# GestaltCogTeam/STEP

Measured on AMD Instinct MI355X. Metric: training windows/sec on PEMS04, horizon-12 MAE parity, 1/2/4/8 MI355X, higher is better.
Workload: dtype f16 (TSFormer Q/K/weights) + bf16 (P, V, GraphWaveNet / graph-learner GEMMs) operands, f32 accumulate

## Files before the change

### step_amd/csrc/gemm.hip

```cpp
#include "common.h"
#include "step_internal.h"

namespace {

constexpr int BK = 32;

template <typename T>
__device__ __forceinline__ float ld_elem(const void* p, long idx) {
    if constexpr (sizeof(T) == 2) {
        return bf16_bits_to_f32(((const uint16_t*)p)[idx]);
    } else {
        return ((const float*)p)[idx];
    }
}

template <int BM, int BN, int WM, int WN, typename TA, typename TB>
__global__ __launch_bounds__(256) void gemm_f32mfma_kernel(StepGemm g) {
    constexpr int TM = BM / WM / 32;
    constexpr int TN = BN / WN / 32;
    constexpr int LDA = BM + 4;
    constexpr int LDB = BN + 4;
    __shared__ __attribute__((aligned(16))) float As[BK * LDA];
    __shared__ __attribute__((aligned(16))) float Bs[BK * LDB];

// ... 396 lines not shown
    }
    if (g.splitk < 1) g.splitk = 1;
    if (g.splitk == 1 && direct_eligible(g)) return launch_direct(g, st);
    if (g.splitk > 1) {
        STEP_REQUIRE(g.accumulate == 2, "step_gemm: split-K needs accumulate==2 (atomic) and a pre-zeroed/accumulating C");
    }
    STEP_REQUIRE(!(g.accumulate == 2 && (g.bias || g.relu)), "step_gemm: bias/relu epilogue not available with atomic accumulate");
    if (g.N <= 32 && g.M > 64) return launch<128, 32, 4, 1>(g, st);
    if (g.M <= 32 && g.N > 64) return launch<32, 128, 1, 4>(g, st);
    if (g.M <= 64 || g.N <= 64) return launch<64, 64, 2, 2>(g, st);
    long tiles128 = (long)cdiv(g.M, 128) * cdiv(g.N, 128) * g.batch * g.splitk;
    if (tiles128 < 256) return launch<64, 64, 2, 2>(g, st);
    return launch<128, 128, 2, 2>(g, st);
}

int step_gemm_launch_fused(StepGemm g, const GemmFused& fused, hipStream_t st) {
    STEP_REQUIRE(g.M > 0 && g.N > 0 && g.K >= 0 && g.batch == 1 && g.A && g.B && g.C, "step_gemm(fused): bad descriptor");
    STEP_REQUIRE(fused.channels > 0 && fused.period > 0 && (long)fused.channels * fused.period == g.N, "step_gemm(fused): N != channels * period");
    if (g.scn == 0) g.scn = 1;
    if (g.splitk < 1) g.splitk = 1;
    if (g.c_nscale) STEP_REQUIRE(g.c_nshift && g.c_mvec && g.c_nperiod == fused.period, "step_gemm(fused): column affine must use the same period");
    if (g.compute_bf16) return step_gemm_bf16_launch(g, st, &fused);
    const int rc = step_gemm_f32_fast_launch(g, st, &fused);
    if (rc == -1) { step_set_error("step_gemm(fused): operands do not qualify for the staged path"); return STEP_ERR_ARG; }
    return rc;
}

extern "C" int step_gemm(const StepGemm* g, void* stream) {
    STEP_REQUIRE(g != nullptr, "step_gemm: null descriptor");
    return step_gemm_launch(*g, (hipStream_t)stream);
// ... 2 lines not shown
```

### step_amd/csrc/gemm_bf16.hip

```cpp
#include "common.h"
#include "step_internal.h"

namespace {

constexpr int BK = 32;
constexpr int PITCH = BK * 2 + 16;

typedef __attribute__((ext_vector_type(4))) float f32x4v;
typedef __attribute__((ext_vector_type(4))) __bf16 bf16x4;

typedef __attribute__((ext_vector_type(2))) float f32x2v;
typedef __attribute__((ext_vector_type(2))) __bf16 bf16x2v;
__device__ __forceinline__ uint32_t pack2(float a, float b) {
    uint32_t r;
    asm("v_cvt_pk_bf16_f32 %0, %1, %2" : "=v"(r) : "v"(a), "v"(b));
    return r;
}
__device__ __forceinline__ uint2 pack4(float a, float b, float c, float d) { return make_uint2(pack2(a, b), pack2(c, d)); }
__device__ __forceinline__ uint2 pack4(const float (&v)[4]) { return pack4(v[0], v[1], v[2], v[3]); }
__device__ __forceinline__ uint16_t bf16_of(float x) {
    return __builtin_bit_cast(uint16_t, (__bf16)x);
}
template <typename T>
__device__ __forceinline__ float ld1(const void* p, long idx) {
// ... 189 lines not shown

enum { KC_F32 = 0, KC_BF16 = 1, MC_F32 = 2, MC_BF16 = 3 };
constexpr int FBK = 64;
constexpr int FPITCH = FBK * 2 + 8;
constexpr int FPITCH32 = FBK * 4 + 16;

struct FastArgs {
    const GemmKSeg* ktab;
    int ktab_per;
    int a_klog, b_klog, b_nlog;
    int xcd_swizzle;
    int wide_store;
    int m_fast;
    long split_stride;
    GemmFused fu;
};

static int wide_store_ok(const StepGemm& g, bool force = false) {
    return g.accumulate != 2 && !g.a_rowsum && g.c_nblk == 0 && g.scn == 1 && g.N % 4 == 0 && g.ldc % 4 == 0 && g.scb % 4 == 0 &&
           g.scb1 % 4 == 0 && ((uintptr_t)g.C & 15) == 0 && (force || (long)g.M * g.N * g.batch >= (4L << 20));
}

__device__ __forceinline__ long remap(int i, int lg, long stride) {
    return (long)(i >> lg) * stride + (i & ((1 << lg) - 1));
}

template <int MODE, int BR>
struct Stage {
    static constexpr int NV = MODE == KC_F32 ? BR * FBK / 4 / 256 : (MODE == KC_BF16 ? BR * FBK / 8 / 256 : (MODE == MC_F32 ? BR * FBK / 16 / 256 : (BR * FBK / 32 + 255) / 256));
    static constexpr int NR = (MODE == MC_F32 || MODE == MC_BF16) ? NV * 4 : NV;
// ... 178 lines not shown
                *(uint2*)(d + (2 * p + 1) * FPITCH) = make_uint2((d0 >> 16) | (d1 & 0xffff0000u), (d2 >> 16) | (d3 & 0xffff0000u));
            }
        }
    } else {
#pragma unroll
        for (int r = 0; r < s.NV; ++r) {
            const int e = tid + r * 256;
            char* d = lds + ((e % (BR / 4)) * 4) * FPITCH + (e / (BR / 4)) * 8;
#pragma unroll
            for (int i = 0; i < 4; ++i)
                *(uint2*)(d + i * FPITCH) = pack4(s.f[r * 4][i], s.f[r * 4 + 1][i], s.f[r * 4 + 2][i], s.f[r * 4 + 3][i]);
        }
    }
}

template <int BM, int BN, int AMODE, int BMODE, bool F32C, bool KTAB = false, bool FUSED = false>
__global__ __launch_bounds__(256) void gemm_fast_kernel(StepGemm g, FastArgs fa) {
    static_assert(!KTAB || (AMODE == KC_F32 && BMODE == KC_F32), "segmented contraction: k-contiguous f32 blocks on both sides");
    constexpr int TM = BM / 64, TN = BN / 64;
    constexpr int PITCH_ = F32C ? FPITCH32 : FPITCH;
    constexpr int BUF = (BM + BN) * PITCH_;
    __shared__ __attribute__((aligned(16))) char lds[2 * BUF];

    const int tid = threadIdx.x, lane = tid & 63, wave = tid >> 6;
    const int wr = wave >> 1, wc = wave & 1;
    unsigned bx = blockIdx.x, by = blockIdx.y, bz = blockIdx.z;
    if (fa.xcd_swizzle) {
        const unsigned gx = gridDim.x, lin = bx + gx * (by + gridDim.y * bz);
        const unsigned q = lin >> 3, j = q / gx, grp = (lin & 7u) + 8u * j;
        bx = q - j * gx; by = grp % gridDim.y; bz = grp / gridDim.y;
    } else if (fa.m_fast) {
// ... 281 lines not shown
            }
        }
        if (fu.dotw) {
            float q4[4] = {dw[0], dm[0], dw[1], dm[1]};
#pragma unroll
            for (int i = 0; i < 4; ++i) q4[i] = wave_sum(q4[i]);
            if (lane == 0) { fred[wave][0] = q4[0]; fred[wave][1] = q4[1]; fred[wave][2] = q4[2]; fred[wave][3] = q4[3]; }
            __syncthreads();
            if (tid < 4) {
                const int c = c_lo + (tid >> 1);
                if (c < C) atomicAdd(fu.dots + 2 * c + (tid & 1), fred[0][tid] + fred[1][tid] + fred[2][tid] + fred[3][tid]);
            }
        }
        return;
    }
    if constexpr (BM * (BN + 4) * 4 <= 2 * BUF)
    if (fa.wide_store) {
        constexpr int TP = BN + 4;
        static_assert(BM * TP * 4 <= 2 * BUF, "staging tile must fit in the operand buffers");
        float* tile = (float*)lds;
        __syncthreads();
#pragma unroll
        for (int i = 0; i < TM; ++i)
#pragma unroll
            for (int j = 0; j < TN; ++j) {
                const int cn = wc * (TN * 32) + j * 32 + r, gn = n0 + cn;
                const GemmColAffine ca = gemm_col_affine(g, gn < g.N ? gn : 0);
                const float bv = (g.bias != nullptr && gn < g.N) ? g.bias[gn] : 0.f;
#pragma unroll
                for (int e = 0; e < 16; ++e) {
// ... 66 lines not shown
    if (bmode == KC_F32) gemm_fast_kernel<BM, BN, AMODE, KC_F32, false><<<grid, 256, 0, st>>>(g, fa);
    else if (bmode == KC_BF16) gemm_fast_kernel<BM, BN, AMODE, KC_BF16, false><<<grid, 256, 0, st>>>(g, fa);
    else if (bmode == MC_F32) gemm_fast_kernel<BM, BN, AMODE, MC_F32, false><<<grid, 256, 0, st>>>(g, fa);
    else {
        if constexpr (AMODE != KC_BF16) gemm_fast_kernel<BM, BN, AMODE, MC_BF16, false><<<grid, 256, 0, st>>>(g, fa);
        else { step_set_error("step_gemm: an n-contiguous bf16 B operand needs an f32 A operand"); return STEP_ERR_ARG; }
    }
    STEP_LAUNCH_CHECK("step_gemm(bf16 fast)");
    return STEP_OK;
}
template <int BM, int BN>
int launch_fast(const StepGemm& g, const FastArgs& fa_in, int amode, int bmode, hipStream_t st) {
    dim3 grid(cdiv(g.N + (g.a_rowsum ? 1 : 0), BN), cdiv(g.M, BM), g.batch * g.splitk);
    FastArgs fa = fa_in;
    fa.xcd_swizzle = grid.x >= 2 && (grid.y * grid.z) % 8 == 0 && (long)g.M * g.K * g.batch >= (8L << 20);
    if (amode == KC_F32) return launch_fast_b<BM, BN, KC_F32>(g, fa, bmode, grid, st);
    if (amode == KC_BF16) return launch_fast_b<BM, BN, KC_BF16>(g, fa, bmode, grid, st);
    return launch_fast_b<BM, BN, MC_F32>(g, fa, bmode, grid, st);
}
template <int BM, int BN>
int launch_fast_fused(const StepGemm& g, const FastArgs& fa_in, int amode, int bmode, hipStream_t st) {
    dim3 grid(cdiv(g.N, BN), cdiv(g.M, BM), 1);
    FastArgs fa = fa_in;
    static const bool m_fast_on = []() { const char* e = getenv("STEP_GEMM_M_FAST"); return !e || atoi(e) != 0; }();
    fa.m_fast = m_fast_on && grid.y >= 2 && grid.y <= 64 && (long)g.N * g.K * (g.b_bf16 ? 2 : 4) >= (16L << 20);
    if (amode == KC_F32 && bmode == MC_BF16) gemm_fast_kernel<BM, BN, KC_F32, MC_BF16, false, false, true><<<grid, 256, 0, st>>>(g, fa);
    else if (amode == KC_F32 && bmode == KC_F32) gemm_fast_kernel<BM, BN, KC_F32, KC_F32, false, false, true><<<grid, 256, 0, st>>>(g, fa);
    else if (amode == KC_F32 && bmode == MC_F32) gemm_fast_kernel<BM, BN, KC_F32, MC_F32, false, false, true><<<grid, 256, 0, st>>>(g, fa);
    else if (amode == MC_F32 && bmode == MC_F32) gemm_fast_kernel<BM, BN, MC_F32, MC_F32, false, false, true><<<grid, 256, 0, st>>>(g, fa);
    else { step_set_error("step_gemm(fused): operand layout not instantiated"); return STEP_ERR_ARG; }
// ... 45 lines not shown
    const long i0 = batch0 ? b % batch0 : b, i1 = batch0 ? b / batch0 : 0;
    atomicAdd(C + i0 * scb + i1 * scb1 + m * ldc + n * scn, s);
}
}

static int auto_splitk(int M, int N, int K, int batch, bool fast) {
    const int bk = fast ? FBK : BK;
    long tiles = fast ? (long)cdiv(M, 128) * cdiv(N, 128) * batch : (long)cdiv(M, 64) * cdiv(N, 64) * batch;
    static const int split_target = []() { const char* e = getenv("STEP_GEMM_SPLIT_TARGET"); return e ? atoi(e) : 768; }();
    long want = ((fast ? split_target : 1024) + tiles - 1) / tiles;
    long maxs = cdiv(K, bk) / 4;
    return (int)(want < 1 ? 1 : (want > maxs ? (maxs < 1 ? 1 : maxs) : want));
}
int step_gemm_auto_splitk(int M, int N, int K, int batch) { return auto_splitk(M, N, K, batch, true); }

int step_gemm_bf16_launch(StepGemm g, hipStream_t st, const GemmFused* fused) {
    FastArgs fa;
    memset(&fa, 0, sizeof(fa));
    if (fused) fa.fu = *fused;
    int dummy;
    const int amode = fast_mode(g.A, g.a_bf16, g.sam, g.sak, g.sab, g.sab1, g.a_kblk, g.a_kstride, 0, 0, &fa.a_klog, &dummy);
    const int bmode = fast_mode(g.B, g.b_bf16, g.sbn, g.sbk, g.sbb, g.sbb1, g.b_kblk, g.b_kstride, g.b_nblk, g.b_nstride, &fa.b_klog,
                                &fa.b_nlog);
    const bool fast = amode >= 0 && amode != MC_BF16 && bmode >= 0 && !(g.a_kscale && (amode != KC_F32 || g.a_kperiod < FBK)) &&
                !(g.a_rowsum && (bmode == KC_BF16 || bmode == MC_BF16)) && !(bmode == MC_BF16 && g.N % 8);
    fa.wide_store = wide_store_ok(g, fused != nullptr);
    if (fused) STEP_REQUIRE(fast && fa.wide_store && !g.bias && !g.relu && g.batch == 1 && g.splitk <= 1 &&
                            ((fused->flags & (GEMM_FUSED_FFN_FWD | GEMM_FUSED_MASKNZ | GEMM_FUSED_BF16OUT)) ? (g.accumulate == 0 && !fused->dotw && !fused->bnx && !g.c_nscale) :
                             (fused->flags & GEMM_FUSED_INTERLEAVED) ? (128 % fused->channels == 0 && fused->channels % 8 == 0 && g.N % 8 == 0 && g.ldc % 8 == 0 &&
                                                                       ((((uintptr_t)fused->bnx) | ((uintptr_t)g.C)) & 15) == 0 && !fused->dotw) : fused->period >= 128),
                            "step_gemm: the fused DGL epilogues need the staged path with a wide-store result (aligned dense C, period >= 128)");
    if (g.splitk < 0) {
        STEP_REQUIRE(g.accumulate == 2, "step_gemm: automatic split-K needs accumulate==2");
        g.splitk = auto_splitk(g.M, g.N, g.K, g.batch, fast);
    }
    if (g.splitk < 1) g.splitk = 1;
    if (g.splitk > 1) STEP_REQUIRE(g.accumulate == 2, "step_gemm: split-K needs accumulate==2");
    STEP_REQUIRE(!(g.accumulate == 2 && (g.bias || g.relu)), "step_gemm: bias/relu epilogue not available with atomic accumulate");
    long tiles128 = (long)cdiv(g.M, 128) * cdiv(g.N, 128) * g.batch * g.splitk;
    const bool big = g.M > 64 && g.N > 64 && tiles128 >= 512;
    static const bool use_ws = []() { const char* e = getenv("STEP_GEMM_SPLITK_WS"); return !e || atoi(e) != 0; }();
    const StepGemm orig = g;
    bool ws_reduce = false;
    if (use_ws && fast && !fused && g.splitk > 1 && g.splitk_ws && !g.c_nblk && !g.c_nscale && (((uintptr_t)g.splitk_ws) & 15) == 0 &&
        (long)g.M * g.N * g.batch * g.splitk <= g.splitk_ws_floats) {
        const long mn = (long)g.M * g.N;
// ... 83 lines not shown
```

### step_amd/csrc/gwnet.hip

```cpp
#include "common.h"
#include "step_internal.h"
#include <vector>

namespace {

constexpr int C = 32, CAT = 224, CS = 256, CE = 512, OUT = 12, NL = 8, HID = 96;
constexpr int TIN[NL] = {13, 12, 10, 9, 7, 6, 4, 3};
constexpr int DIL[NL] = {1, 2, 1, 2, 1, 2, 1, 2};
constexpr int TOUT[NL] = {12, 10, 9, 7, 6, 4, 3, 1};

__global__ void start_conv_kernel(const float* __restrict__ hist, int B, int N, int Cin, const float* __restrict__ w,
                                  const float* __restrict__ b, float* __restrict__ x0) {
    long idx = (long)blockIdx.x * 256 + threadIdx.x;
    long total = (long)B * N * 13 * C;
    if (idx >= total) return;
    int c = idx % C, t = (idx / C) % 13;
    long bn = idx / (C * 13);
    int n = bn % N, bb = bn / N;
    float v = b[c];
    if (t >= 1) {
        const float* src = hist + (((long)bb * 12 + (t - 1)) * N + n) * Cin;
        v += w[c * 2] * src[0] + w[c * 2 + 1] * src[1];
    }
    x0[idx] = v;
// ... 86 lines not shown
}
__global__ void stacks_to_bf16_kernel(const float* __restrict__ P, const float* __restrict__ PT, long rows, int N, int N8,
                                      uint16_t* __restrict__ P16, uint16_t* __restrict__ PT16) {
    long idx = (long)blockIdx.x * 256 + threadIdx.x;
    if (idx >= rows * (N8 / 2)) return;
    const long row = idx / (N8 / 2);
    const int j = (int)(idx % (N8 / 2)) * 2;
    const float* src = blockIdx.y ? PT : P;
    uint16_t* dst = blockIdx.y ? PT16 : P16;
    const float a = j < N ? src[row * N + j] : 0.f, b = j + 1 < N ? src[row * N + j + 1] : 0.f;
    typedef __attribute__((ext_vector_type(2))) float f2;
    typedef __attribute__((ext_vector_type(2))) __bf16 b2;
    f2 t = {a, b};
    *(uint32_t*)(dst + row * N8 + j) = __builtin_bit_cast(uint32_t, __builtin_convertvector(t, b2));
}
__global__ __launch_bounds__(256) void slots_to_bf16T_kernel(const float* __restrict__ cat, int slot0, int sstep, int B, int N, int T, int N8,
                                                             uint16_t* __restrict__ XT) {
    __shared__ float tile[64][33];
    const int v0 = blockIdx.x * 64, t = blockIdx.y, src = blockIdx.z / B, b = blockIdx.z % B;
    const int slot = slot0 + sstep * src;
    const int c = threadIdx.x & 31, r = threadIdx.x >> 5;
    for (int i = r; i < 64; i += 8) {
        const int v = v0 + i;
        tile[i][c] = v < N ? cat[(((long)b * N + v) * T + t) * CAT + slot * C + c] : 0.f;
    }
    __syncthreads();
    const int cc = threadIdx.x >> 3, g8 = (threadIdx.x & 7) * 8;
    if (v0 + g8 < N8) {
        float v8[8];
#pragma unroll
        for (int j = 0; j < 8; ++j) v8[j] = tile[g8 + j][cc];
        *(bf16x8*)(XT + (((long)blockIdx.z * T + t) * C + cc) * N8 + v0 + g8) = pack8(v8);
    }
}
__global__ void sum_batches_kernel(const float* __restrict__ x, long n, int B, float* __restrict__ out) {
    long idx = (long)blockIdx.x * 256 + threadIdx.x;
    if (idx >= n) return;
    float s = 0.f;
    for (int b = 0; b < B; ++b) s += x[(long)b * n + idx];
    out[idx] = s;
}
__global__ __launch_bounds__(256) void row_dot_kernel(const float* __restrict__ dP, const float* __restrict__ P, int N,
                                                      float* __restrict__ out) {
    __shared__ float red[4];
    const long row = blockIdx.x;
    float s = 0.f;
    for (int j = threadIdx.x; j < N; j += 256) s += dP[row * N + j] * P[row * N + j];
    s = wave_sum(s);
// ... 170 lines not shown
    __shared__ double tot[64];
    if (threadIdx.x < 64) tot[threadIdx.x] = gather_sum(bn.sums, threadIdx.x);
    __syncthreads();
    if (threadIdx.x < 32) {
        const int c = threadIdx.x;
        co[c] = (float)(tot[c] / bn.count); co[32 + c] = (float)(tot[32 + c] / bn.count); co[64 + c] = bn.gamma[c] * bn.stat[96 + c];
        if (blockIdx.x == 0) { bn.dgamma[c] += (float)tot[32 + c]; bn.dbeta[c] += (float)tot[c]; }
    }
    __syncthreads();
}

template <bool BF16>
__global__ __launch_bounds__(256) void tcn_fwd_kernel(const float* __restrict__ src, BnFwd bn, long npos, int Tin, int Tout, int dil,
                                                      const float* __restrict__ wcat, const float* __restrict__ bcat,
                                                      float* __restrict__ tf, float* __restrict__ sg, float* __restrict__ cat,
                                                      float* __restrict__ zlast, int layer) {
    __shared__ float st[128];
    if (bn.stat) bn_fwd_stats(bn, st);
    const int lane = threadIdx.x & 63, wave = threadIdx.x >> 6, col = lane & 31, h = lane >> 5;
    const long r0 = ((long)blockIdx.x * 4 + wave) * 32;
    if (r0 >= npos) return;
    long p = r0 + col;
    if (p >= npos) p = npos - 1;
    const long bn_ = p / Tout;
    const long xrow = bn_ * Tin + (p - bn_ * Tout);
    float a[4][8], bf[4][8], bg[4][8];
#pragma unroll
    for (int q = 0; q < 4; ++q) {
        load8h(src + (xrow + (q >> 1) * dil) * C + 16 * (q & 1), h, a[q]);
        load8h(wcat + col * 64 + 16 * q, h, bf[q]);
        load8h(wcat + (32 + col) * 64 + 16 * q, h, bg[q]);
    }
    if (bn.stat) {
#pragma unroll
        for (int q = 0; q < 4; ++q)
#pragma unroll
            for (int j = 0; j < 8; ++j) { const int c = chan8h(q & 1, h, j); a[q][j] = a[q][j] * st[c] + st[32 + c]; }
    }
    f32x16 af, ag;
#pragma unroll
    for (int e = 0; e < 16; ++e) { af[e] = 0.f; ag[e] = 0.f; }
#pragma unroll
    for (int q = 0; q < 4; ++q) { mma16<BF16>(af, a[q], bf[q]); mma16<BF16>(ag, a[q], bg[q]); }
    const float b_f = bcat[col], b_g = bcat[32 + col];
#pragma unroll
    for (int e = 0; e < 16; ++e) {
        const long pe = r0 + (e & 3) + 8 * (e >> 2) + 4 * h;
        if (pe >= npos) continue;
        const float f = tanhf(af[e] + b_f);
        const float g = 1.f / (1.f + __expf(-(ag[e] + b_g)));
        tf[pe * C + col] = f; sg[pe * C + col] = g;
        cat[pe * CAT + col] = f * g;
        const long bne = pe / Tout;
        if (pe - bne * Tout == Tout - 1) zlast[bne * CS + layer * C + col] = f * g;
    }
}

template <bool BF16>
__global__ __launch_bounds__(256) void mix_fwd_kernel(const float* __restrict__ cat, const float* __restrict__ w,
                                                      const float* __restrict__ bias, XIn x, long npos, int Tin, int Tout, int dil,
                                                      float drop_p, uint32_t seed_lo, uint32_t seed_hi, uint32_t layer,
                                                      float* __restrict__ mask, float* __restrict__ y, double* __restrict__ sums,
                                                      const StepDynState* __restrict__ dyn) {
    if (dyn) { const uint64_t sx = dyn->seed_xor; seed_lo ^= (uint32_t)sx; seed_hi ^= (uint32_t)(sx >> 32); }
    __shared__ float red[4][64];
    __shared__ float bsum[64];
    const int lane = threadIdx.x & 63, wave = threadIdx.x >> 6, ln = lane & 15, kg = lane >> 4;
    const long r0 = ((long)blockIdx.x * 4 + wave) * 16;
    float s1[2] = {0.f, 0.f}, s2[2] = {0.f, 0.f};
    if (r0 < npos) {
// ... 49 lines not shown
        for (int half = 0; half < 2; ++half) {
            s1[half] += __shfl_xor(s1[half], 16, 64); s2[half] += __shfl_xor(s2[half], 16, 64);
            s1[half] += __shfl_xor(s1[half], 32, 64); s2[half] += __shfl_xor(s2[half], 32, 64);
        }
    }
    if (kg == 0) { red[wave][ln] = s1[0]; red[wave][16 + ln] = s1[1]; red[wave][32 + ln] = s2[0]; red[wave][48 + ln] = s2[1]; }
    __syncthreads();
    if (threadIdx.x < 64) bsum[threadIdx.x] = red[0][threadIdx.x] + red[1][threadIdx.x] + red[2][threadIdx.x] + red[3][threadIdx.x];
    __syncthreads();
    add_block_sums(sums, bsum);
}

template <bool BF16>
__global__ __launch_bounds__(256) void mix_bwd_kernel(const float* __restrict__ dy, const float* __restrict__ y, BnBwd bn,
                                                      const float* __restrict__ mask, const float* __restrict__ wT, long npos,
                                                      float* __restrict__ dres, float* __restrict__ dh, float* __restrict__ dcat) {
    __shared__ float co[96];
    bn_bwd_coef(bn, co);
    const int lane = threadIdx.x & 63, wave = threadIdx.x >> 6, col = lane & 31, h = lane >> 5;
    const long r0 = ((long)blockIdx.x * 4 + wave) * 32;
    if (r0 >= npos) return;
    const long p = r0 + col;
    const bool ok = p < npos;
    float a[2][8];
#pragma unroll
    for (int q = 0; q < 2; ++q) {
        float d8[8] = {0.f, 0.f, 0.f, 0.f, 0.f, 0.f, 0.f, 0.f}, y8[8] = {0.f, 0.f, 0.f, 0.f, 0.f, 0.f, 0.f, 0.f}, m8[8] = {1.f, 1.f, 1.f, 1.f, 1.f, 1.f, 1.f, 1.f};
        if (ok) {
            load8h(dy + p * C + 16 * q, h, d8); load8h(y + p * C + 16 * q, h, y8);
            if (mask) load8h(mask + p * C + 16 * q, h, m8);
        }
#pragma unroll
        for (int j = 0; j < 8; ++j) {
            const int c = chan8h(q, h, j);
            const float xhat = (y8[j] - bn.stat[64 + c]) * bn.stat[96 + c];
            const float d = ok ? co[64 + c] * (d8[j] - co[c] - xhat * co[32 + c]) : 0.f;
            d8[j] = d;
            a[q][j] = d * m8[j];
        }
        if (ok) { store8h(dres + p * C + 16 * q, h, d8); store8h(dh + p * C + 16 * q, h, a[q]); }
    }
#pragma unroll
    for (int slot = 0; slot < 7; ++slot) {
        float b[2][8];
#pragma unroll
        for (int q = 0; q < 2; ++q) load8h(wT + (slot * C + col) * C + 16 * q, h, b[q]);
        f32x16 acc;
#pragma unroll
        for (int e = 0; e < 16; ++e) acc[e] = 0.f;
#pragma unroll
        for (int q = 0; q < 2; ++q) mma16<BF16>(acc, a[q], b[q]);
#pragma unroll
        for (int e = 0; e < 16; ++e) {
            const long pe = r0 + (e & 3) + 8 * (e >> 2) + 4 * h;
            if (pe < npos) dcat[pe * CAT + slot * C + col] = acc[e];
        }
    }
}

constexpr int TB_ROWS = 64;
template <bool BF16>
__global__ __launch_bounds__(256) void tcn_bwd_kernel(const float* __restrict__ dcat, const float* __restrict__ dzlast, int layer,
                                                      const float* __restrict__ tf, const float* __restrict__ sg,
                                                      const float* __restrict__ wcatT, const float* __restrict__ dres, long BN, int Tin,
                                                      int Tout, int dil, float* __restrict__ dpre, float* __restrict__ dx,
                                                      const float* __restrict__ yprev, const float* __restrict__ statprev,
                                                      double* __restrict__ sums) {
    __shared__ float dxs[TB_ROWS][65];
    __shared__ float red[8][64];
    __shared__ float bsum[64];
    const int G = TB_ROWS / Tout, R = G * Tout;
// ... 147 lines not shown
inline dim3 g1(long n) { return dim3((unsigned)((n + 255) / 256)); }

struct Carver {
    float* base;
    long used = 0;
    explicit Carver(float* b) : base(b) {}
    float* take(long n) {
        float* p = base ? base + used : nullptr;
        used += (n + 3) & ~3L;
        return p;
    }
};

static inline int n8(int N) { return (N + 7) & ~7; }
static inline bool hop_transposed_operand(int N) {
    static const int min_n = []() { const char* e = getenv("STEP_HOP_XT_MIN_N"); return e ? atoi(e) : 768; }();
    return N >= min_n;
}

struct Saved {
    float *x0, *cat[NL], *tf[NL], *sg[NL], *y[NL], *mask[NL], *bnstat[NL], *zlast;
    float *Pstk, *PTstk, *Pa, *Madp, *rs, *cs;
    uint16_t *P16, *PT16;
    float *skip, *h1, *h2, *xh, *e1;
    long total;
};
Saved carve_saved(float* base, int B, int N, bool dropout) {
    Carver cv(base);
    Saved s;
    const long BN = (long)B * N;
    s.x0 = cv.take(BN * TIN[0] * C);
// ... 14 lines not shown
    s.Madp = cv.take((long)N * N);
    s.rs = cv.take(BN);
    s.cs = cv.take(BN);
    s.skip = cv.take(BN * CS);
    s.h1 = cv.take(BN * CE);
    s.h2 = cv.take(BN * CS);
    s.xh = cv.take(BN * CS);
    s.e1 = cv.take(BN * CE);
    s.total = cv.used;
    return s;
}
struct Work {
    float *wcat, *wcatT, *bcat, *wskip, *wmixT, *dwcat, *dbcat, *dwskip;
    double* acc64;
    float *xcat[NL], *bsum, *y7, *m7;
    uint16_t* xT;
    float *dcat[NL - 1], *dpre[NL], *dh[NL - 1], *dres, *dxa, *dxb, *dskip, *dPstk, *dPa, *dM, *rf, *rb;
    GemmKSeg* ktab;
    float *d_e1, *d_xh, *d_h2, *d_h1;
    long total;
};
Work carve_work(float* base, int B, int N, bool backward) {
    Carver cv(base);
    Work w;
    const long BN = (long)B * N;
    w.wcat = cv.take(NL * 64 * 64);
    w.wcatT = cv.take(NL * 64 * 64);
    w.bcat = cv.take(NL * 64);
    w.wskip = cv.take(CS * CS);
    w.wmixT = cv.take(7 * C * CAT);
    w.dwcat = cv.take(NL * 64 * 64);
    w.dbcat = cv.take(NL * 64);
    w.dwskip = cv.take(CS * CS);
    w.acc64 = (double*)cv.take(2L * NL * NCOPY * 64);
    w.xT = hop_transposed_operand(N) ? (uint16_t*)cv.take(3L * B * 12 * C * n8(N) / 2) : nullptr;
    for (int i = 0; i < NL; ++i) w.xcat[i] = backward ? cv.take(BN * TOUT[i] * 64) : nullptr;
    w.bsum = cv.take(CS);
    w.y7 = cv.take(BN * TOUT[NL - 1] * C);
    w.m7 = cv.take(BN * TOUT[NL - 1] * C);
    if (backward) {
        for (int i = 0; i < NL - 1; ++i) w.dcat[i] = cv.take(BN * TOUT[i] * CAT);
        w.ktab = (GemmKSeg*)cv.take(3L * ADJ_NSEG * sizeof(GemmKSeg) / sizeof(float));
        for (int i = 0; i < NL; ++i) w.dpre[i] = cv.take(BN * TOUT[i] * 64);
        for (int i = 0; i < NL - 1; ++i) w.dh[i] = cv.take(BN * TOUT[i] * C);
        w.dres = cv.take(BN * 12 * C);
        w.dxa = cv.take(BN * 13 * C);
        w.dxb = cv.take(BN * 13 * C);
        w.dskip = cv.take(BN * CS);
        w.dPstk = cv.take(3L * B * N * N);
        w.dPa = cv.take((long)N * N);
// ... 5 lines not shown
        w.d_h2 = cv.take(BN * CS);
        w.d_h1 = cv.take(BN * CE);
    }
    w.total = cv.used;
    return w;
}

int zero(float* p, long n, hipStream_t st) {
    if (hipMemsetAsync(p, 0, (size_t)n * sizeof(float), st) != hipSuccess) {
        step_set_error("gwnet: memset failed");
        return STEP_ERR_HIP;
    }
    return STEP_OK;
}

int nconv_fwd3(const float* Pstk, const uint16_t* PT16, float* cat, int src0, int sstep, int dst0, int B, int N, int T, int bf16,
               uint16_t* xT, hipStream_t st) {
    StepGemm g = gemm_desc(N, T * C, N, Pstk, 1, N, cat + src0 * C, (long)T * CAT, 1, cat + dst0 * C, (long)T * CAT);
    if (bf16 && xT) {
        const int nsrc = sstep == 0 ? 1 : 3;
        slots_to_bf16T_kernel<<<dim3(cdiv(N, 64), T, nsrc * B), 256, 0, st>>>(cat, src0, sstep, B, N, T, n8(N), xT);
        STEP_LAUNCH_CHECK("slots_to_bf16T");
        g.batch = 3 * B; g.batch0 = B;
        g.A = PT16; g.a_bf16 = 1; g.sam = n8(N); g.sak = 1; g.sab = (long)N * n8(N); g.sab1 = (long)B * N * n8(N);
        g.B = xT; g.b_bf16 = 1; g.sbk = 1; g.sbn = n8(N); g.sbb = (long)T * C * n8(N); g.sbb1 = nsrc == 1 ? 0 : (long)B * T * C * n8(N);
        g.scb = (long)N * T * CAT; g.scb1 = 2L * C;
        g.c_nblk = C; g.c_nstride = CAT;
        g.compute_bf16 = 1;
        return step_gemm_launch(g, st);
    }
    g.batch = 3 * B; g.batch0 = B;
    g.sab = (long)N * N; g.sab1 = (long)B * N * N;
    if (bf16) { g.A = PT16; g.a_bf16 = 1; g.sam = n8(N); g.sak = 1; g.sab = (long)N * n8(N); g.sab1 = (long)B * N * n8(N); }
    g.sbb = (long)N * T * CAT; g.sbb1 = (long)sstep * C;
    g.scb = (long)N * T * CAT; g.scb1 = 2L * C;
    g.b_nblk = C; g.b_nstride = CAT; g.c_nblk = C; g.c_nstride = CAT;
    g.compute_bf16 = bf16;
    return step_gemm_launch(g, st);
}
int nconv_bwd_data3(const float* PTstk, const uint16_t* P16, float* dcat, int src0, int dst0, int dstep, int B, int N, int T, int bf16,
                    uint16_t* xT, hipStream_t st) {
    StepGemm g = gemm_desc(N, T * C, N, PTstk, 1, N, dcat + src0 * C, (long)T * CAT, 1, dcat + dst0 * C, (long)T * CAT);
    if (bf16 && xT) {
        slots_to_bf16T_kernel<<<dim3(cdiv(N, 64), T, 3 * B), 256, 0, st>>>(dcat, src0, 2, B, N, T, n8(N), xT);
        STEP_LAUNCH_CHECK("slots_to_bf16T");
        g.batch = 3 * B; g.batch0 = B;
        g.A = P16; g.a_bf16 = 1; g.sam = n8(N); g.sak = 1; g.sab = (long)N * n8(N); g.sab1 = (long)B * N * n8(N);
        g.B = xT; g.b_bf16 = 1; g.sbk = 1; g.sbn = n8(N); g.sbb = (long)T * C * n8(N); g.sbb1 = (long)B * T * C * n8(N);
        g.scb = (long)N * T * CAT; g.scb1 = (long)dstep * C;
        g.c_nblk = C; g.c_nstride = CAT;
        g.accumulate = dstep == 0 ? 2 : 1;
        g.compute_bf16 = 1;
        return step_gemm_launch(g, st);
    }
    g.batch = 3 * B; g.batch0 = B;
    g.sab = (long)N * N; g.sab1 = (long)B * N * N;
    if (bf16) { g.A = P16; g.a_bf16 = 1; g.sam = n8(N); g.sak = 1; g.sab = (long)N * n8(N); g.sab1 = (long)B * N * n8(N); }
    g.sbb = (long)N * T * CAT; g.sbb1 = 2L * C;
    g.scb = (long)N * T * CAT; g.scb1 = (long)dstep * C;
    g.b_nblk = C; g.b_nstride = CAT; g.c_nblk = C; g.c_nstride = CAT;
    g.accumulate = dstep == 0 ? 2 : 1;
    g.compute_bf16 = bf16;
    return step_gemm_launch(g, st);
}
}

extern "C" long step_gwnet_saved_floats(int B, int N, int dropout) { return carve_saved(nullptr, B, N, dropout != 0).total; }
extern "C" long step_gwnet_work_floats(int B, int N, int backward) { return carve_work(nullptr, B, N, backward != 0).total; }
// ... 4 lines not shown
}

template <bool BF16>
static int gwnet_layers_forward(const StepGwnetParams* p, const Saved& S, const Work& W, int B, int N, bool training, float drop_p,
                                uint64_t seed, float momentum, bool dead_bn7, const StepDynState* dyn, hipStream_t st,
                                bool first_tcn_only = false, bool skip_first_tcn = false) {
    const long BN = (long)B * N;
    for (int i = 0; i < (first_tcn_only ? 1 : NL); ++i) {
        const int Tin = TIN[i], Tout = TOUT[i], dil = DIL[i];
        const long npos = BN * Tout;
        BnFwd bn = {nullptr, nullptr, nullptr, nullptr, training ? 1 : 0, momentum, nullptr, (double)BN * Tin, nullptr};
        if (i > 0) {
            bn.gamma = p->bn_w[i - 1]; bn.beta = p->bn_b[i - 1]; bn.rm = p->bn_rm[i - 1]; bn.rv = p->bn_rv[i - 1];
            bn.stat = S.bnstat[i - 1]; bn.sums = W.acc64 + (long)(i - 1) * NCOPY * 64;
        }
        if (!(i == 0 && skip_first_tcn)) {
            tcn_fwd_kernel<BF16><<<(unsigned)cdiv(npos, 128), 256, 0, st>>>(i == 0 ? S.x0 : S.y[i - 1], bn, npos, Tin, Tout, dil, W.wcat + i * 4096,
                                                                            W.bcat + i * 64, S.tf[i], S.sg[i], S.cat[i], S.zlast, i);
            STEP_LAUNCH_CHECK("tcn_fwd");
        }
        if (first_tcn_only) break;
        if (i == NL - 1 && !(dead_bn7 && training)) break;
        STEP_TRY(nconv_fwd3(S.Pstk, S.PT16, S.cat[i], 0, 0, 1, B, N, Tout, BF16, W.xT, st));
        STEP_TRY(nconv_fwd3(S.Pstk, S.PT16, S.cat[i], 1, 2, 2, B, N, Tout, BF16, W.xT, st));
        const XIn xin = {i == 0 ? S.x0 : S.y[i - 1], i == 0 ? nullptr : S.bnstat[i - 1]};
        const bool dead = i == NL - 1;
        mix_fwd_kernel<BF16><<<(unsigned)cdiv(npos, 64), 256, 0, st>>>(S.cat[i], p->gconv_w[i], p->gconv_b[i], xin, npos, Tin, Tout, dil, drop_p,
                                                                       (uint32_t)seed, (uint32_t)(seed >> 32), (uint32_t)i, dead ? W.m7 : S.mask[i],
                                                                       dead ? W.y7 : S.y[i], W.acc64 + (long)i * NCOPY * 64, dyn);
        STEP_LAUNCH_CHECK("mix_fwd");
        if (dead) {
            const BnFwd b7 = {p->bn_w[i], p->bn_b[i], p->bn_rm[i], p->bn_rv[i], 1, momentum, S.bnstat[i], (double)npos, W.acc64 + (long)i * NCOPY * 64};
            bn_stats_only_kernel<<<1, 64, 0, st>>>(b7);
            STEP_LAUNCH_CHECK("bn7_stats");
        }
    }
    return STEP_OK;
}

// ... 125 lines not shown
        for (int i = lo; i <= hi; ++i) nseg += 2 * TOUT[i];
        StepGemm g = gemm_desc(N, N, 32 * nseg, S.cat[0], 0, 1, W.dcat[0], 1, 0, W.dPstk, N);
        g.batch = 3 * B; g.batch0 = B;
        g.scb = (long)N * N; g.scb1 = (long)B * N * N;
        g.compute_bf16 = BF16;
        g.accumulate = adj_first ? 0 : 1;
        adj_first = false;
        return step_gemm_segmented_launch(g, W.ktab + seg0, ADJ_NSEG, on_stream);
    };
    for (int i = NL - 1; i >= 0; --i) {
        const int Tin = TIN[i], Tout = TOUT[i], dil = DIL[i];
        const long npos = BN * Tout;
        const float* cat = S.cat[i];
        if (i < NL - 1) {
            const BnBwd bn = {p->bn_w[i], S.bnstat[i], grads->bn_w[i], grads->bn_b[i], (double)npos, W.acc64 + (long)i * NCOPY * 64};
            mix_bwd_kernel<BF16><<<(unsigned)cdiv(npos, 128), 256, 0, st>>>(dx_next, S.y[i], bn, S.mask[i], W.wmixT + i * (C * CAT), npos, W.dres, W.dh[i],
                                                                            W.dcat[i]);
            STEP_LAUNCH_CHECK("mix_bwd");
            STEP_TRY(nconv_bwd_data3(S.PTstk, S.P16, W.dcat[i], 2, 1, 2, B, N, Tout, BF16, W.xT, st));
            STEP_TRY(nconv_bwd_data3(S.PTstk, S.P16, W.dcat[i], 1, 0, 0, B, N, Tout, BF16, W.xT, st));
            if (adj_pieces && i == 0) { STEP_TRY(adj_piece(0, 0, lane.fork())); *adj_done = lane.done(); }
        }
        float* dx = dxbuf[i & 1];
        tcn_bwd_kernel<BF16><<<(unsigned)cdiv(BN, TB_ROWS / Tout), 256, 0, st>>>(i < NL - 1 ? W.dcat[i] : nullptr, W.dskip, i, S.tf[i], S.sg[i],
                                                                                W.wcatT + i * 4096, i < NL - 1 ? W.dres : nullptr, BN, Tin, Tout, dil,
                                                                                W.dpre[i], dx, i > 0 ? S.y[i - 1] : nullptr,
                                                                                i > 0 ? S.bnstat[i - 1] : nullptr,
                                                                                i > 0 ? W.acc64 + (long)(i - 1) * NCOPY * 64 : nullptr);
        STEP_LAUNCH_CHECK("tcn_bwd");
        const XIn xin = {i == 0 ? S.x0 : S.y[i - 1], i == 0 ? nullptr : S.bnstat[i - 1]};
        hipEvent_t ev = leaves.on ? leaves.mark() : lane.mark();
        if (adj_pieces && i == 4) STEP_TRY(adj_piece(4, 6, lane.after(ev)));
        if (adj_pieces && i == 2) STEP_TRY(adj_piece(2, 3, lane.after(ev)));
        if (adj_pieces && i == 1) STEP_TRY(adj_piece(1, 1, lane.after(ev)));
        hipStream_t leaf = leaves.after(ev);
// ... 128 lines not shown
```

### step_amd/csrc/step_internal.h

```cpp
#pragma once
#include <hip/hip_runtime.h>
#include <vector>
#include "../../include/step_hip.h"

enum { GEMM_FUSED_INTERLEAVED = 1, GEMM_FUSED_FFN_FWD = 2, GEMM_FUSED_MASKNZ = 4, GEMM_FUSED_BF16OUT = 8 };
struct GemmFused {
    const float* dotw; float* dots;
    const float* bnx; const float* bncoef; const float* bnstat;
    int channels, period;
    int flags;
    const float* ffn_bias; const void* maskx; float p; unsigned seed_lo, seed_hi, site;
};

struct GemmKSeg { long a_off, b_off, a_bs, b_bs; int a_rs, b_rs; };
constexpr int GEMM_KSEG_MAX = 128;
int step_gemm_segmented_launch(StepGemm g, const GemmKSeg* ktab, int ktab_per, hipStream_t st);

int step_gemm_launch(StepGemm g, hipStream_t st);
int step_gemm_auto_splitk(int M, int N, int K, int batch);
int step_gemm_launch_fused(StepGemm g, const GemmFused& fused, hipStream_t st);
int step_gemm_bf16_launch(StepGemm g, hipStream_t st, const GemmFused* fused = nullptr);
int step_gemm_f32_fast_launch(StepGemm g, hipStream_t st, const GemmFused* fused = nullptr);

static inline StepGemm gemm_desc(int M, int N, int K, const float* A, long sam, long sak, const float* B, long sbk,
                                 long sbn, float* C, long ldc) {
    StepGemm g;
    memset(&g, 0, sizeof(g));
    g.M = M; g.N = N; g.K = K; g.batch = 1;
    g.A = A; g.sam = sam; g.sak = sak;
    g.B = B; g.sbk = sbk; g.sbn = sbn;
    g.C = C; g.ldc = ldc; g.scn = 1;
    g.alpha = 1.f; g.splitk = 1;
    return g;
}

int step_gemm_rowsum_separate(StepGemm* g, hipStream_t st);
// ... 79 lines not shown
```

Baseline: 2364.

## Fuse transposed bf16 hop operand emission into producer kernels and GEMM epilogues

Removes the standalone slots_to_bf16T transpose kernel. The transposed bf16 diffusion-hop operand is now written directly by tcn_fwd and mix_bwd, which remap their waves to node-major tiles, and by a new EMIT epilogue in the bf16 GEMM that stores a packed transposed copy for the next hop. Two xT buffers are ping-ponged. The default threshold for using the transposed operand drops from N>=768 to 0, so PEMS04 (307 nodes) now takes this path. Risks: strided row mapping in tcn/mix kernels can hurt coalescing, and the EMIT epilogue drops wide stores.

```diff
diff --git a/step_amd/csrc/gemm.hip b/step_amd/csrc/gemm.hip
--- a/step_amd/csrc/gemm.hip
+++ b/step_amd/csrc/gemm.hip
@@ -434,6 +434,13 @@
     return launch<128, 128, 2, 2>(g, st);
 }
 
+int step_gemm_launch_emit(StepGemm g, const GemmEmit& emit, hipStream_t st) {
+    STEP_REQUIRE(g.M > 0 && g.N > 0 && g.K >= 0 && g.batch > 0 && g.A && g.B && g.C, "step_gemm(emit): bad descriptor");
+    STEP_REQUIRE(g.compute_bf16 && g.a_bf16 && g.b_bf16, "step_gemm(emit): bf16 operands only");
+    if (g.scn == 0) g.scn = 1;
+    return step_gemm_bf16_launch(g, st, nullptr, &emit);
+}
+
 int step_gemm_launch_fused(StepGemm g, const GemmFused& fused, hipStream_t st) {
     STEP_REQUIRE(g.M > 0 && g.N > 0 && g.K >= 0 && g.batch == 1 && g.A && g.B && g.C, "step_gemm(fused): bad descriptor");
     STEP_REQUIRE(fused.channels > 0 && fused.period > 0 && (long)fused.channels * fused.period == g.N, "step_gemm(fused): N != channels * period");
diff --git a/step_amd/csrc/gemm_bf16.hip b/step_amd/csrc/gemm_bf16.hip
--- a/step_amd/csrc/gemm_bf16.hip
+++ b/step_amd/csrc/gemm_bf16.hip
@@ -227,6 +227,7 @@
     int m_fast;
     long split_stride;
     GemmFused fu;
+    GemmEmit emit;
 };
 
 static int wide_store_ok(const StepGemm& g, bool force = false) {
@@ -435,7 +436,7 @@
     }
 }
 
-template <int BM, int BN, int AMODE, int BMODE, bool F32C, bool KTAB = false, bool FUSED = false>
+template <int BM, int BN, int AMODE, int BMODE, bool F32C, bool KTAB = false, bool FUSED = false, bool EMIT = false>
 __global__ __launch_bounds__(256) void gemm_fast_kernel(StepGemm g, FastArgs fa) {
     static_assert(!KTAB || (AMODE == KC_F32 && BMODE == KC_F32), "segmented contraction: k-contiguous f32 blocks on both sides");
     constexpr int TM = BM / 64, TN = BN / 64;
@@ -747,6 +748,44 @@
         }
         return;
     }
+    if constexpr (EMIT) {
+        static_assert(!F32C && !KTAB && !FUSED, "the transposed copy belongs to the plain bf16 kernels");
+        uint16_t* Eb = fa.emit.dst + (long)i0 * fa.emit.sb0 + (long)i1 * fa.emit.sb1;
+#pragma unroll
+        for (int i = 0; i < TM; ++i)
+#pragma unroll
+            for (int j = 0; j < TN; ++j) {
+                const int gn = n0 + wc * (TN * 32) + j * 32 + r;
+                const int mb = m0 + wr * (TM * 32) + i * 32 + 4 * h;
+                if (gn >= g.N) continue;
+                const long ni = g.c_nblk ? (long)(gn / g.c_nblk) * g.c_nstride + (gn % g.c_nblk) : (long)gn;
+                float* col = Cb + ni * g.scn;
+                float v[16];
+                if (g.accumulate == 1) {
+                    float old[16];
+#pragma unroll
+                    for (int e = 0; e < 16; ++e) {
+                        const int gm = mb + (e & 3) + 8 * (e >> 2);
+                        old[e] = gm < g.M ? col[(long)gm * g.ldc] : 0.f;
+                    }
+#pragma unroll
+                    for (int e = 0; e < 16; ++e) v[e] = g.alpha * acc[i][j][e] + old[e] + 0.f;
+                } else {
+#pragma unroll
+                    for (int e = 0; e < 16; ++e) v[e] = g.alpha * acc[i][j][e] + 0.f;
+                }
+#pragma unroll
+                for (int e = 0; e < 16; ++e) {
+                    const int gm = mb + (e & 3) + 8 * (e >> 2);
+                    if (gm < g.M) col[(long)gm * g.ldc] = v[e]; else v[e] = 0.f;
+                }
+                uint16_t* ecol = Eb + (long)gn * fa.emit.pitch;
+#pragma unroll
+                for (int q = 0; q < 4; ++q)
+                    if (mb + 8 * q < g.M) *(uint2*)(ecol + mb + 8 * q) = pack4(v[4 * q], v[4 * q + 1], v[4 * q + 2], v[4 * q + 3]);
+            }
+        return;
+    }
     if constexpr (BM * (BN + 4) * 4 <= 2 * BUF)
     if (fa.wide_store) {
         constexpr int TP = BN + 4;
@@ -843,6 +882,11 @@
     dim3 grid(cdiv(g.N + (g.a_rowsum ? 1 : 0), BN), cdiv(g.M, BM), g.batch * g.splitk);
     FastArgs fa = fa_in;
     fa.xcd_swizzle = grid.x >= 2 && (grid.y * grid.z) % 8 == 0 && (long)g.M * g.K * g.batch >= (8L << 20);
+    if (fa.emit.dst) {
+        gemm_fast_kernel<BM, BN, KC_BF16, KC_BF16, false, false, false, true><<<grid, 256, 0, st>>>(g, fa);
+        STEP_LAUNCH_CHECK("step_gemm(bf16 fast, transposed copy)");
+        return STEP_OK;
+    }
     if (amode == KC_F32) return launch_fast_b<BM, BN, KC_F32>(g, fa, bmode, grid, st);
     if (amode == KC_BF16) return launch_fast_b<BM, BN, KC_BF16>(g, fa, bmode, grid, st);
     return launch_fast_b<BM, BN, MC_F32>(g, fa, bmode, grid, st);
@@ -918,10 +962,11 @@
 }
 int step_gemm_auto_splitk(int M, int N, int K, int batch) { return auto_splitk(M, N, K, batch, true); }
 
-int step_gemm_bf16_launch(StepGemm g, hipStream_t st, const GemmFused* fused) {
+int step_gemm_bf16_launch(StepGemm g, hipStream_t st, const GemmFused* fused, const GemmEmit* emit) {
     FastArgs fa;
     memset(&fa, 0, sizeof(fa));
     if (fused) fa.fu = *fused;
+    if (emit) fa.emit = *emit;
     int dummy;
     const int amode = fast_mode(g.A, g.a_bf16, g.sam, g.sak, g.sab, g.sab1, g.a_kblk, g.a_kstride, 0, 0, &fa.a_klog, &dummy);
     const int bmode = fast_mode(g.B, g.b_bf16, g.sbn, g.sbk, g.sbb, g.sbb1, g.b_kblk, g.b_kstride, g.b_nblk, g.b_nstride, &fa.b_klog,
@@ -934,6 +979,14 @@
                              (fused->flags & GEMM_FUSED_INTERLEAVED) ? (128 % fused->channels == 0 && fused->channels % 8 == 0 && g.N % 8 == 0 && g.ldc % 8 == 0 &&
                                                                        ((((uintptr_t)fused->bnx) | ((uintptr_t)g.C)) & 15) == 0 && !fused->dotw) : fused->period >= 128),
                             "step_gemm: the fused DGL epilogues need the staged path with a wide-store result (aligned dense C, period >= 128)");
+    if (emit) {
+        STEP_REQUIRE(fast && !fused && amode == KC_BF16 && bmode == KC_BF16 && g.accumulate != 2 && g.splitk == 1 && !g.bias && !g.relu &&
+                     !g.c_nscale && !g.a_rowsum,
+                     "step_gemm(emit): needs the staged path with k-contiguous bf16 operands and a plain store / += epilogue");
+        STEP_REQUIRE(emit->dst && ((uintptr_t)emit->dst & 7) == 0 && emit->pitch % 8 == 0 && emit->pitch >= ((g.M + 3) & ~3) &&
+                     emit->sb0 % 4 == 0 && emit->sb1 % 4 == 0, "step_gemm(emit): bad layout of the transposed copy");
+        fa.wide_store = 0;
+    }
     if (g.splitk < 0) {
         STEP_REQUIRE(g.accumulate == 2, "step_gemm: automatic split-K needs accumulate==2");
         g.splitk = auto_splitk(g.M, g.N, g.K, g.batch, fast);
diff --git a/step_amd/csrc/gwnet.hip b/step_amd/csrc/gwnet.hip
--- a/step_amd/csrc/gwnet.hip
+++ b/step_amd/csrc/gwnet.hip
@@ -124,24 +124,34 @@
     f2 t = {a, b};
     *(uint32_t*)(dst + row * N8 + j) = __builtin_bit_cast(uint32_t, __builtin_convertvector(t, b2));
 }
-__global__ __launch_bounds__(256) void slots_to_bf16T_kernel(const float* __restrict__ cat, int slot0, int sstep, int B, int N, int T, int N8,
-                                                             uint16_t* __restrict__ XT) {
-    __shared__ float tile[64][33];
-    const int v0 = blockIdx.x * 64, t = blockIdx.y, src = blockIdx.z / B, b = blockIdx.z % B;
-    const int slot = slot0 + sstep * src;
-    const int c = threadIdx.x & 31, r = threadIdx.x >> 5;
-    for (int i = r; i < 64; i += 8) {
-        const int v = v0 + i;
-        tile[i][c] = v < N ? cat[(((long)b * N + v) * T + t) * CAT + slot * C + c] : 0.f;
-    }
-    __syncthreads();
-    const int cc = threadIdx.x >> 3, g8 = (threadIdx.x & 7) * 8;
-    if (v0 + g8 < N8) {
-        float v8[8];
-#pragma unroll
-        for (int j = 0; j < 8; ++j) v8[j] = tile[g8 + j][cc];
-        *(bf16x8*)(XT + (((long)blockIdx.z * T + t) * C + cc) * N8 + v0 + g8) = pack8(v8);
-    }
+struct HopXT { uint16_t* p; int N, N8; };
+typedef __attribute__((ext_vector_type(4))) __bf16 bf16x4_t;
+__device__ __forceinline__ uint2 pack4_bf16(const float* v) {
+    const f32x4 t = {v[0], v[1], v[2], v[3]};
+    return __builtin_bit_cast(uint2, __builtin_convertvector(t, bf16x4_t));
+}
+struct RowMap { long r0, step, bt; int nvalid, node0; };
+__device__ __forceinline__ bool wave_rows(const HopXT& x, long tile, long npos, int T, RowMap& m) {
+    if (!x.p) {
+        m.r0 = tile * 32; m.step = 1; m.bt = 0; m.node0 = 0;
+        if (m.r0 >= npos) return false;
+        m.nvalid = (int)(npos - m.r0 < 32 ? npos - m.r0 : 32);
+        return true;
+    }
+    const int ntile = (x.N + 31) >> 5;
+    m.bt = tile / ntile;
+    m.node0 = (int)(tile - m.bt * ntile) * 32;
+    const long b = m.bt / T;
+    if (b * x.N * T >= npos) return false;
+    m.r0 = (b * x.N + m.node0) * T + (m.bt - b * T); m.step = T;
+    m.nvalid = x.N - m.node0 < 32 ? x.N - m.node0 : 32;
+    return true;
+}
+__device__ __forceinline__ void store_xt(const HopXT& x, const RowMap& m, long npos, int src, int col, int h, const float* v) {
+    uint16_t* d = x.p + ((src * (npos / x.N) + m.bt) * C + col) * x.N8 + m.node0 + 4 * h;
+#pragma unroll
+    for (int q = 0; q < 4; ++q)
+        if (m.node0 + 4 * h + 8 * q < x.N) *(uint2*)(d + 8 * q) = pack4_bf16(v + 4 * q);
 }
 __global__ void sum_batches_kernel(const float* __restrict__ x, long n, int B, float* __restrict__ out) {
     long idx = (long)blockIdx.x * 256 + threadIdx.x;
@@ -342,14 +352,13 @@
 __global__ __launch_bounds__(256) void tcn_fwd_kernel(const float* __restrict__ src, BnFwd bn, long npos, int Tin, int Tout, int dil,
                                                       const float* __restrict__ wcat, const float* __restrict__ bcat,
                                                       float* __restrict__ tf, float* __restrict__ sg, float* __restrict__ cat,
-                                                      float* __restrict__ zlast, int layer) {
+                                                      float* __restrict__ zlast, int layer, HopXT xt) {
     __shared__ float st[128];
     if (bn.stat) bn_fwd_stats(bn, st);
     const int lane = threadIdx.x & 63, wave = threadIdx.x >> 6, col = lane & 31, h = lane >> 5;
-    const long r0 = ((long)blockIdx.x * 4 + wave) * 32;
-    if (r0 >= npos) return;
-    long p = r0 + col;
-    if (p >= npos) p = npos - 1;
+    RowMap rm;
+    if (!wave_rows(xt, (long)blockIdx.x * 4 + wave, npos, Tout, rm)) return;
+    const long p = rm.r0 + (col < rm.nvalid ? col : rm.nvalid - 1) * rm.step;
     const long bn_ = p / Tout;
     const long xrow = bn_ * Tin + (p - bn_ * Tout);
     float a[4][8], bf[4][8], bg[4][8];
@@ -371,17 +380,22 @@
 #pragma unroll
     for (int q = 0; q < 4; ++q) { mma16<BF16>(af, a[q], bf[q]); mma16<BF16>(ag, a[q], bg[q]); }
     const float b_f = bcat[col], b_g = bcat[32 + col];
+    float z[16];
 #pragma unroll
     for (int e = 0; e < 16; ++e) {
-        const long pe = r0 + (e & 3) + 8 * (e >> 2) + 4 * h;
-        if (pe >= npos) continue;
+        const int row = (e & 3) + 8 * (e >> 2) + 4 * h;
+        z[e] = 0.f;
+        if (row >= rm.nvalid) continue;
+        const long pe = rm.r0 + row * rm.step;
         const float f = tanhf(af[e] + b_f);
         const float g = 1.f / (1.f + __expf(-(ag[e] + b_g)));
+        z[e] = f * g;
         tf[pe * C + col] = f; sg[pe * C + col] = g;
-        cat[pe * CAT + col] = f * g;
+        cat[pe * CAT + col] = z[e];
         const long bne = pe / Tout;
-        if (pe - bne * Tout == Tout - 1) zlast[bne * CS + layer * C + col] = f * g;
-    }
+        if (pe - bne * Tout == Tout - 1) zlast[bne * CS + layer * C + col] = z[e];
+    }
+    if (xt.p) store_xt(xt, rm, npos, 0, col, h, z);
 }
 
 template <bool BF16>
@@ -461,14 +475,15 @@
 template <bool BF16>
 __global__ __launch_bounds__(256) void mix_bwd_kernel(const float* __restrict__ dy, const float* __restrict__ y, BnBwd bn,
                                                       const float* __restrict__ mask, const float* __restrict__ wT, long npos,
-                                                      float* __restrict__ dres, float* __restrict__ dh, float* __restrict__ dcat) {
+                                                      float* __restrict__ dres, float* __restrict__ dh, float* __restrict__ dcat, int T,
+                                                      HopXT xt) {
     __shared__ float co[96];
     bn_bwd_coef(bn, co);
     const int lane = threadIdx.x & 63, wave = threadIdx.x >> 6, col = lane & 31, h = lane >> 5;
-    const long r0 = ((long)blockIdx.x * 4 + wave) * 32;
-    if (r0 >= npos) return;
-    const long p = r0 + col;
-    const bool ok = p < npos;
+    RowMap rm;
+    if (!wave_rows(xt, (long)blockIdx.x * 4 + wave, npos, T, rm)) return;
+    const long p = rm.r0 + col * rm.step;
+    const bool ok = col < rm.nvalid;
     float a[2][8];
 #pragma unroll
     for (int q = 0; q < 2; ++q) {
@@ -497,11 +512,14 @@
         for (int e = 0; e < 16; ++e) acc[e] = 0.f;
 #pragma unroll
         for (int q = 0; q < 2; ++q) mma16<BF16>(acc, a[q], b[q]);
+        float v[16];
 #pragma unroll
         for (int e = 0; e < 16; ++e) {
-            const long pe = r0 + (e & 3) + 8 * (e >> 2) + 4 * h;
-            if (pe < npos) dcat[pe * CAT + slot * C + col] = acc[e];
-        }
+            const int row = (e & 3) + 8 * (e >> 2) + 4 * h;
+            v[e] = row < rm.nvalid ? acc[e] : 0.f;
+            if (row < rm.nvalid) dcat[(rm.r0 + row * rm.step) * CAT + slot * C + col] = acc[e];
+        }
+        if (xt.p && slot >= 2 && (slot & 1) == 0) store_xt(xt, rm, npos, (slot - 2) >> 1, col, h, v);
     }
 }
 
@@ -679,7 +697,7 @@
 
 static inline int n8(int N) { return (N + 7) & ~7; }
 static inline bool hop_transposed_operand(int N) {
-    static const int min_n = []() { const char* e = getenv("STEP_HOP_XT_MIN_N"); return e ? atoi(e) : 768; }();
+    static const int min_n = []() { const char* e = getenv("STEP_HOP_XT_MIN_N"); return e ? atoi(e) : 0; }();
     return N >= min_n;
 }
 
@@ -724,7 +742,7 @@
     float *wcat, *wcatT, *bcat, *wskip, *wmixT, *dwcat, *dbcat, *dwskip;
     double* acc64;
     float *xcat[NL], *bsum, *y7, *m7;
-    uint16_t* xT;
+    uint16_t* xT[2];
     float *dcat[NL - 1], *dpre[NL], *dh[NL - 1], *dres, *dxa, *dxb, *dskip, *dPstk, *dPa, *dM, *rf, *rb;
     GemmKSeg* ktab;
     float *d_e1, *d_xh, *d_h2, *d_h1;
@@ -743,7 +761,7 @@
     w.dbcat = cv.take(NL * 64);
     w.dwskip = cv.take(CS * CS);
     w.acc64 = (double*)cv.take(2L * NL * NCOPY * 64);
-    w.xT = hop_transposed_operand(N) ? (uint16_t*)cv.take(3L * B * 12 * C * n8(N) / 2) : nullptr;
+    for (int k = 0; k < 2; ++k) w.xT[k] = hop_transposed_operand(N) ? (uint16_t*)cv.take(3L * B * 12 * C * n8(N) / 2) : nullptr;
     for (int i = 0; i < NL; ++i) w.xcat[i] = backward ? cv.take(BN * TOUT[i] * 64) : nullptr;
     w.bsum = cv.take(CS);
     w.y7 = cv.take(BN * TOUT[NL - 1] * C);
@@ -779,20 +797,21 @@
     return STEP_OK;
 }
 
+static inline GemmEmit hop_emit(uint16_t* xT_out, int B, int N, int T) {
+    return GemmEmit{xT_out, (long)T * C * n8(N), (long)B * T * C * n8(N), n8(N)};
+}
 int nconv_fwd3(const float* Pstk, const uint16_t* PT16, float* cat, int src0, int sstep, int dst0, int B, int N, int T, int bf16,
-               uint16_t* xT, hipStream_t st) {
+               const uint16_t* xT, uint16_t* xT_out, hipStream_t st) {
     StepGemm g = gemm_desc(N, T * C, N, Pstk, 1, N, cat + src0 * C, (long)T * CAT, 1, cat + dst0 * C, (long)T * CAT);
     if (bf16 && xT) {
         const int nsrc = sstep == 0 ? 1 : 3;
-        slots_to_bf16T_kernel<<<dim3(cdiv(N, 64), T, nsrc * B), 256, 0, st>>>(cat, src0, sstep, B, N, T, n8(N), xT);
-        STEP_LAUNCH_CHECK("slots_to_bf16T");
         g.batch = 3 * B; g.batch0 = B;
         g.A = PT16; g.a_bf16 = 1; g.sam = n8(N); g.sak = 1; g.sab = (long)N * n8(N); g.sab1 = (long)B * N * n8(N);
         g.B = xT; g.b_bf16 = 1; g.sbk = 1; g.sbn = n8(N); g.sbb = (long)T * C * n8(N); g.sbb1 = nsrc == 1 ? 0 : (long)B * T * C * n8(N);
         g.scb = (long)N * T * CAT; g.scb1 = 2L * C;
         g.c_nblk = C; g.c_nstride = CAT;
         g.compute_bf16 = 1;
-        return step_gemm_launch(g, st);
+        return xT_out ? step_gemm_launch_emit(g, hop_emit(xT_out, B, N, T), st) : step_gemm_launch(g, st);
     }
     g.batch = 3 * B; g.batch0 = B;
     g.sab = (long)N * N; g.sab1 = (long)B * N * N;
@@ -804,11 +823,9 @@
     return step_gemm_launch(g, st);
 }
 int nconv_bwd_data3(const float* PTstk, const uint16_t* P16, float* dcat, int src0, int dst0, int dstep, int B, int N, int T, int bf16,
-                    uint16_t* xT, hipStream_t st) {
+                    const uint16_t* xT, uint16_t* xT_out, hipStream_t st) {
     StepGemm g = gemm_desc(N, T * C, N, PTstk, 1, N, dcat + src0 * C, (long)T * CAT, 1, dcat + dst0 * C, (long)T * CAT);
     if (bf16 && xT) {
-        slots_to_bf16T_kernel<<<dim3(cdiv(N, 64), T, 3 * B), 256, 0, st>>>(dcat, src0, 2, B, N, T, n8(N), xT);
-        STEP_LAUNCH_CHECK("slots_to_bf16T");
         g.batch = 3 * B; g.batch0 = B;
         g.A = P16; g.a_bf16 = 1; g.sam = n8(N); g.sak = 1; g.sab = (long)N * n8(N); g.sab1 = (long)B * N * n8(N);
         g.B = xT; g.b_bf16 = 1; g.sbk = 1; g.sbn = n8(N); g.sbb = (long)T * C * n8(N); g.sbb1 = (long)B * T * C * n8(N);
@@ -816,7 +833,7 @@
         g.c_nblk = C; g.c_nstride = CAT;
         g.accumulate = dstep == 0 ? 2 : 1;
         g.compute_bf16 = 1;
-        return step_gemm_launch(g, st);
+        return xT_out ? step_gemm_launch_emit(g, hop_emit(xT_out, B, N, T), st) : step_gemm_launch(g, st);
     }
     g.batch = 3 * B; g.batch0 = B;
     g.sab = (long)N * N; g.sab1 = (long)B * N * N;
@@ -851,15 +868,18 @@
             bn.gamma = p->bn_w[i - 1]; bn.beta = p->bn_b[i - 1]; bn.rm = p->bn_rm[i - 1]; bn.rv = p->bn_rv[i - 1];
             bn.stat = S.bnstat[i - 1]; bn.sums = W.acc64 + (long)(i - 1) * NCOPY * 64;
         }
+        const bool gcn = !(i == NL - 1 && !(dead_bn7 && training));
+        const HopXT xt = {BF16 && gcn ? W.xT[0] : nullptr, N, n8(N)};
         if (!(i == 0 && skip_first_tcn)) {
-            tcn_fwd_kernel<BF16><<<(unsigned)cdiv(npos, 128), 256, 0, st>>>(i == 0 ? S.x0 : S.y[i - 1], bn, npos, Tin, Tout, dil, W.wcat + i * 4096,
-                                                                            W.bcat + i * 64, S.tf[i], S.sg[i], S.cat[i], S.zlast, i);
+            const long tiles = xt.p ? (long)B * Tout * cdiv(N, 32) : cdiv(npos, 32);
+            tcn_fwd_kernel<BF16><<<(unsigned)cdiv(tiles, 4), 256, 0, st>>>(i == 0 ? S.x0 : S.y[i - 1], bn, npos, Tin, Tout, dil, W.wcat + i * 4096,
+                                                                           W.bcat + i * 64, S.tf[i], S.sg[i], S.cat[i], S.zlast, i, xt);
             STEP_LAUNCH_CHECK("tcn_fwd");
         }
         if (first_tcn_only) break;
-        if (i == NL - 1 && !(dead_bn7 && training)) break;
-        STEP_TRY(nconv_fwd3(S.Pstk, S.PT16, S.cat[i], 0, 0, 1, B, N, Tout, BF16, W.xT, st));
-        STEP_TRY(nconv_fwd3(S.Pstk, S.PT16, S.cat[i], 1, 2, 2, B, N, Tout, BF16, W.xT, st));
+        if (!gcn) break;
+        STEP_TRY(nconv_fwd3(S.Pstk, S.PT16, S.cat[i], 0, 0, 1, B, N, Tout, BF16, W.xT[0], W.xT[1], st));
+        STEP_TRY(nconv_fwd3(S.Pstk, S.PT16, S.cat[i], 1, 2, 2, B, N, Tout, BF16, W.xT[1], nullptr, st));
         const XIn xin = {i == 0 ? S.x0 : S.y[i - 1], i == 0 ? nullptr : S.bnstat[i - 1]};
         const bool dead = i == NL - 1;
         mix_fwd_kernel<BF16><<<(unsigned)cdiv(npos, 64), 256, 0, st>>>(S.cat[i], p->gconv_w[i], p->gconv_b[i], xin, npos, Tin, Tout, dil, drop_p,
@@ -1015,11 +1035,13 @@
         const float* cat = S.cat[i];
         if (i < NL - 1) {
             const BnBwd bn = {p->bn_w[i], S.bnstat[i], grads->bn_w[i], grads->bn_b[i], (double)npos, W.acc64 + (long)i * NCOPY * 64};
-            mix_bwd_kernel<BF16><<<(unsigned)cdiv(npos, 128), 256, 0, st>>>(dx_next, S.y[i], bn, S.mask[i], W.wmixT + i * (C * CAT), npos, W.dres, W.dh[i],
-                                                                            W.dcat[i]);
+            const HopXT xt = {BF16 ? W.xT[0] : nullptr, N, n8(N)};
+            const long tiles = xt.p ? (long)B * Tout * cdiv(N, 32) : cdiv(npos, 32);
+            mix_bwd_kernel<BF16><<<(unsigned)cdiv(tiles, 4), 256, 0, st>>>(dx_next, S.y[i], bn, S.mask[i], W.wmixT + i * (C * CAT), npos, W.dres, W.dh[i],
+                                                                           W.dcat[i], Tout, xt);
             STEP_LAUNCH_CHECK("mix_bwd");
-            STEP_TRY(nconv_bwd_data3(S.PTstk, S.P16, W.dcat[i], 2, 1, 2, B, N, Tout, BF16, W.xT, st));
-            STEP_TRY(nconv_bwd_data3(S.PTstk, S.P16, W.dcat[i], 1, 0, 0, B, N, Tout, BF16, W.xT, st));
+            STEP_TRY(nconv_bwd_data3(S.PTstk, S.P16, W.dcat[i], 2, 1, 2, B, N, Tout, BF16, W.xT[0], W.xT[1], st));
+            STEP_TRY(nconv_bwd_data3(S.PTstk, S.P16, W.dcat[i], 1, 0, 0, B, N, Tout, BF16, W.xT[1], nullptr, st));
             if (adj_pieces && i == 0) { STEP_TRY(adj_piece(0, 0, lane.fork())); *adj_done = lane.done(); }
         }
         float* dx = dxbuf[i & 1];
diff --git a/step_amd/csrc/step_internal.h b/step_amd/csrc/step_internal.h
--- a/step_amd/csrc/step_internal.h
+++ b/step_amd/csrc/step_internal.h
@@ -12,6 +12,8 @@
     const float* ffn_bias; const void* maskx; float p; unsigned seed_lo, seed_hi, site;
 };
 
+struct GemmEmit { uint16_t* dst; long sb0, sb1; int pitch; };
+
 struct GemmKSeg { long a_off, b_off, a_bs, b_bs; int a_rs, b_rs; };
 constexpr int GEMM_KSEG_MAX = 128;
 int step_gemm_segmented_launch(StepGemm g, const GemmKSeg* ktab, int ktab_per, hipStream_t st);
@@ -19,7 +21,8 @@
 int step_gemm_launch(StepGemm g, hipStream_t st);
 int step_gemm_auto_splitk(int M, int N, int K, int batch);
 int step_gemm_launch_fused(StepGemm g, const GemmFused& fused, hipStream_t st);
-int step_gemm_bf16_launch(StepGemm g, hipStream_t st, const GemmFused* fused = nullptr);
+int step_gemm_launch_emit(StepGemm g, const GemmEmit& emit, hipStream_t st);
+int step_gemm_bf16_launch(StepGemm g, hipStream_t st, const GemmFused* fused = nullptr, const GemmEmit* emit = nullptr);
 int step_gemm_f32_fast_launch(StepGemm g, hipStream_t st, const GemmFused* fused = nullptr);
 
 static inline StepGemm gemm_desc(int M, int N, int K, const float* A, long sam, long sak, const float* B, long sbk,
```

New measurement: 2365, median of 6. No clear change (+0.1%).
